# cristicbz/rust-doom

Measured on NVIDIA H100. Metric: frames/sec at 1920x1080 (palette-index bit-exact), higher is better.
Workload: dtype u8

## Files before the change

### rust-doom_b200/csrc/b2d_kernels.cu

```cuda
#include <type_traits>

#include "b2d_kernels.cuh"

namespace b2d {

namespace {

constexpr unsigned kFull = 0xFFFFFFFFu;

constexpr int kMaskWords = 128;
constexpr int kStackDepth = 128;

constexpr uint32_t kVisBit = 1u << 25, kSolidBit = 1u << 24;
__device__ __forceinline__ uint32_t pack_range(int lo, int hi, uint32_t bits) {
    return (uint32_t)lo | ((uint32_t)hi << 12) | bits;
}
__device__ __forceinline__ int range_lo(uint32_t r) { return (int)(r & 0xFFFu); }
__device__ __forceinline__ int range_hi(uint32_t r) { return (int)((r >> 12) & 0xFFFu); }

__device__ __forceinline__ uint32_t word_bits(int w, int lo, int hi) {
    int a = max(lo, w * 32), b = min(hi, w * 32 + 31);
    if (a > b) return 0u;
    uint32_t m = 0xFFFFFFFFu >> (31 - (b - w * 32));
    return m & (0xFFFFFFFFu << (a - w * 32));
// ... 331 lines not shown
    const uint8_t *texels, *flats;
    int row;
};

struct RasterCtx {
    const DeviceScene *sc;
    FixedWarp fix;
    uint32_t pal_s;
    uint2 *rowz;
    PlaneDir dir;
    uint8_t *fb;
    uint32_t *rgba;
    int W, H, x, lane;
    uint32_t skycol;
};

template <bool kRgba>
__device__ __forceinline__ void put_px(const RasterCtx &c, uint8_t *p8, uint32_t *p32, bool on, uint32_t v) {
    if (on) {
        if (kRgba) {
            *p8 = (uint8_t)v;
            *p32 = lds_u32(c.pal_s + 4u * v);
        } else {
            __stcs(p8, (uint8_t)v);
        }
    }
}

__host__ __device__ __forceinline__ bool tex_interleaved(const TexRec &T) { return b2d::tex_interleaved(T.h, T.texel_off); }

constexpr int kBatch = 8;

template <bool kRgba, int kW>
__device__ __forceinline__ void store_batch(const RasterCtx &c, uint8_t *p8, uint32_t *p32, const uint32_t (&v)[kBatch],
                                            int y, int ya, int yb, bool full) {
    const int Wc = kW ? kW : c.W;
    if (full) {
#pragma unroll
        for (int k = 0; k < kBatch; k++) put_px<kRgba>(c, p8 + (size_t)k * Wc, kRgba ? p32 + (size_t)k * Wc : nullptr, true, v[k]);
    } else {
        const uint32_t m = row_mask(y, ya, yb, kBatch);
#pragma unroll
        for (int k = 0; k < kBatch; k++)
            put_px<kRgba>(c, p8 + (size_t)k * Wc, kRgba ? p32 + (size_t)k * Wc : nullptr, (m >> k) & 1u, v[k]);
    }
}

template <bool kRgba, int kW>
__device__ __forceinline__ void fill_void_warp(const RasterCtx &c, int ya, int yb) {
    bool act = ya < yb;
    int y0 = __reduce_min_sync(kFull, act ? ya : 0x7FFFFFFF);
    int y1 = __reduce_max_sync(kFull, act ? yb : 0);
    if (y0 >= y1) return;
    const int Wc = kW ? kW : c.W;
    uint8_t *p8 = c.fb + (size_t)y0 * Wc;
    uint32_t *p32 = kRgba ? c.rgba + (size_t)y0 * Wc : nullptr;
#pragma unroll 1
    for (int y = y0; y < y1; y++, p8 += Wc, p32 += Wc) put_px<kRgba>(c, p8, p32, y >= ya && y < yb, 0u);
}

template <bool kRgba, int kW>
__device__ __forceinline__ void draw_sky_warp(const RasterCtx &c, int ya, int yb) {
    const DeviceScene &sc = *c.sc;
    if (sc.sky_tex < 0) { fill_void_warp<kRgba, kW>(c, ya, yb); return; }
    const TexRec T = sc.tex[sc.sky_tex];
    const bool inter = tex_interleaved(T);
    const uint8_t *px = sc.lit_texels + T.texel_off + (inter ? 4u * c.skycol : c.skycol);
    const uint32_t w4 = 4u * T.w;
    bool act = ya < yb;
    int y0 = __reduce_min_sync(kFull, act ? ya : 0x7FFFFFFF);
    int y1 = __reduce_max_sync(kFull, act ? yb : 0);
    if (y0 >= y1) return;
    const int Wc = kW ? kW : c.W;
    uint8_t *p8 = c.fb + (size_t)y0 * Wc;
    uint32_t *p32 = kRgba ? c.rgba + (size_t)y0 * Wc : nullptr;
#pragma unroll 2
    for (int y = y0; y < y1; y++, p8 += Wc, p32 += Wc) {
        const uint32_t r = sc.skyrow[y];
        put_px<kRgba>(c, p8, p32, y >= ya && y < yb, __ldg(px + (inter ? (r >> 2) * w4 + (r & 3u) : r * T.w)));
    }
}

template <bool kRgba, int kW, bool kFixed = false>
__device__ __forceinline__ void draw_plane_warp(const RasterCtx &c, const FrameConst &fc, const View &vw,
                                                int ya, int yb, int32_t h, int32_t flat, int lightb,
                                                bool visible) {
    const DeviceScene &sc = *c.sc;
    if (!__any_sync(kFull, ya < yb)) return;
    if (!visible) { fill_void_warp<kRgba, kW>(c, ya, yb); return; }
    if (flat == kFlatSky) { draw_sky_warp<kRgba, kW>(c, ya, yb); return; }
    if (flat < 0 || flat >= sc.nflats) { fill_void_warp<kRgba, kW>(c, ya, yb); return; }
    const uint8_t *lit_flats = sc.lit_flats;
    int fixed_row = -1;
    if constexpr (kFixed) {
        lit_flats = c.fix.row == 32 ? c.fix.flats : lit_flats;
        fixed_row = c.fix.row == 32 ? 0 : c.fix.row;
    }
    const uint64_t px_hi = reinterpret_cast<uint64_t>(lit_flats) & 0xFFFFFFFF00000000ull;
    const uint32_t habs = plane_habs(h, fc.pose.z);
    bool act = ya < yb;
    int y0 = __reduce_min_sync(kFull, act ? ya : 0x7FFFFFFF);
    int y1 = __reduce_max_sync(kFull, act ? yb : 0);
    const int full_lo = __reduce_max_sync(kFull, act ? ya : 0x7FFFFFFF);
    const int full_hi = __reduce_min_sync(kFull, act ? yb : 0);
    const int Wc = kW ? kW : c.W;
    uint8_t *p8 = c.fb + (size_t)y0 * Wc;
    uint32_t *p32 = kRgba ? c.rgba + (size_t)y0 * Wc : nullptr;
    const uint32_t bu = (uint32_t)fc.pose.x << 10, bv = (uint32_t)fc.pose.y << 10;
    const uint32_t ax = (uint32_t)c.dir.ax, ay = (uint32_t)c.dir.ay;
    for (int yc = y0; yc < y1; yc += 32) {
        int yy = yc + c.lane;
        if (yy < y1) {
            const PlaneRow pr = plane_row(habs, sc.yslope[yy]);
            c.rowz[c.lane] = make_uint2(pr.z8q, (sc.lit_flat_stride >> 6) * (uint32_t)(kFixed && fixed_row >= 0 ? fixed_row : light_row(lightb, pr.z8)) + 64u * (uint32_t)flat);
        }
        __syncwarp();
        const int rows = min(32, y1 - yc);
        int j = 0;
        for (; j + kBatch <= rows; j += kBatch, p8 += (size_t)kBatch * Wc, p32 += (size_t)kBatch * Wc) {
            uint32_t v[kBatch];
#pragma unroll
            for (int k = 0; k < kBatch; k++) {
                const uint2 rz = c.rowz[j + k];
                v[k] = __ldg(reinterpret_cast<const uint8_t *>(px_hi | flat_offset(rz.y, bu + rz.x * ax, bv + rz.x * ay)));
            }
            const int y = yc + j;
            store_batch<kRgba, kW>(c, p8, p32, v, y, ya, yb, y >= full_lo && y + kBatch <= full_hi);
        }
        for (; j < rows; j++, p8 += Wc, p32 += Wc) {
            const uint2 rz = c.rowz[j];
            const int y = yc + j;
            put_px<kRgba>(c, p8, p32, y >= ya && y < yb,
                          __ldg(reinterpret_cast<const uint8_t *>(px_hi | flat_offset(rz.y, bu + rz.x * ax, bv + rz.x * ay))));
        }
        __syncwarp();
    }
}

template <bool kRgba, int kW, int R>
__device__ __forceinline__ void wall_fast_loop(const RasterCtx &c, const uint8_t *plq, uint32_t w4, uint32_t nq, uint32_t q,
                                               uint32_t acc, uint32_t ts29, int y0, int y1, int ya, int yb,
                                               int full_lo, int full_hi) {
    const int Wc = kW ? kW : c.W;
    uint8_t *p8 = c.fb + (size_t)y0 * Wc;
    uint32_t *p32 = kRgba ? c.rgba + (size_t)y0 * Wc : nullptr;
    asm("" : "+l"(plq));
#pragma unroll 1
    for (int y = y0; y < y1; y += R, p8 += (size_t)R * Wc, p32 += (size_t)R * Wc) {
        const uint32_t q1 = q + 1u == nq ? 0u : q + 1u;
        const uint32_t w0 = __ldg(reinterpret_cast<const uint32_t *>(plq + (size_t)q * w4));
        const uint32_t w1 = __ldg(reinterpret_cast<const uint32_t *>(plq + (size_t)q1 * w4));
        if (y >= full_lo && y + R <= full_hi) {
#pragma unroll
            for (int k = 0; k < R; k++) {
                uint32_t v = pick_byte(w0, w1, wall_sel(acc, ts29, (uint32_t)k));
                if (kRgba) v &= 0xFFu;
                put_px<kRgba>(c, p8 + (size_t)k * Wc, kRgba ? p32 + (size_t)k * Wc : nullptr, true, v);
            }
        } else {
            const uint32_t m = row_mask(y, ya, yb, R);
#pragma unroll
            for (int k = 0; k < R; k++) {
                uint32_t v = pick_byte(w0, w1, wall_sel(acc, ts29, (uint32_t)k));
                if (kRgba) v &= 0xFFu;
                put_px<kRgba>(c, p8 + (size_t)k * Wc, kRgba ? p32 + (size_t)k * Wc : nullptr, (m >> k) & 1u, v);
            }
        }
        wall_advance(acc, q, ts29, (uint32_t)R, nq);
    }
}

template <bool kRgba, int kW, bool kFixed = false>
__device__ __forceinline__ void draw_wall_warp(const RasterCtx &c, const FrameConst &fc, int ya, int yb,
                                               int32_t tex, int32_t tA, int32_t hA, int32_t ucol,
                                               int32_t iscale, int row) {
    const DeviceScene &sc = *c.sc;
    if (!__any_sync(kFull, ya < yb)) return;
    if (tex < 0 || tex >= sc.ntex) { fill_void_warp<kRgba, kW>(c, ya, yb); return; }
    const TexRec T = sc.tex[tex];
    bool act = ya < yb;
    const uint32_t col = (uint32_t)floormod32(ucol, (int32_t)T.w);
    const uint8_t *pl = sc.lit_texels + (size_t)row * sc.lit_texel_stride + T.texel_off;
    if constexpr (kFixed) {
        if (row == 32) pl = c.fix.texels + T.texel_off;
    }
    const uint32_t tstep = (uint32_t)(iscale >> 4);
    int y0 = __reduce_min_sync(kFull, act ? ya : 0x7FFFFFFF);
    int y1 = __reduce_max_sync(kFull, act ? yb : 0);
    const int full_lo = __reduce_max_sync(kFull, act ? ya : 0x7FFFFFFF);
    const int full_hi = __reduce_min_sync(kFull, act ? yb : 0);
    uint32_t t = (uint32_t)wall_tbase(tA, hA, fc.pose.z, c.H, iscale) + (uint32_t)y0 * tstep;
    const int Wc = kW ? kW : c.W;
    uint8_t *p8 = c.fb + (size_t)y0 * Wc;
    uint32_t *p32 = kRgba ? c.rgba + (size_t)y0 * Wc : nullptr;
    if (tex_interleaved(T) && T.h >= 8u) {
        const uint32_t ts = act ? tstep : 0u;
        const bool f16 = __all_sync(kFull, ts <= kWallFast16);
        if (f16 || __all_sync(kFull, ts <= kWallFast8)) {
            const uint32_t tt = act ? t : 0u;
            const uint32_t r0 = wall_row((int32_t)tt, T.h, T.hmagic, T.hbias);
            const uint8_t *plq = pl + 4u * col;
            if (f16) wall_fast_loop<kRgba, kW, 16>(c, plq, 4u * T.w, T.h >> 2, r0 >> 2, wall_acc29(tt, r0), ts << 13, y0, y1, ya, yb, full_lo, full_hi);
            else wall_fast_loop<kRgba, kW, 8>(c, plq, 4u * T.w, T.h >> 2, r0 >> 2, wall_acc29(tt, r0), ts << 13, y0, y1, ya, yb, full_lo, full_hi);
            return;
        }
    }
    if (tex_interleaved(T)) {
        const uint32_t colb = 4u * col, w4 = 4u * T.w;
        for (int y = y0; y < y1; y += kBatch, p8 += (size_t)kBatch * Wc, p32 += (size_t)kBatch * Wc, t += (uint32_t)kBatch * tstep) {
            const uint32_t r0 = wall_row((int32_t)t, T.h, T.hmagic, T.hbias);
            const uint32_t acc = wall_acc(t, r0);
            const uint32_t b7 = (acc + 7u * tstep) >> 16;
            uint32_t v[kBatch];
            if (__all_sync(kFull, b7 < 8u)) {
                const uint32_t q0 = r0 >> 2, q1 = next_quad(q0, T.h);
                const uint32_t w0 = __ldg(reinterpret_cast<const uint32_t *>(pl + (q0 * w4 + colb)));
                const uint32_t w1 = __ldg(reinterpret_cast<const uint32_t *>(pl + (q1 * w4 + colb)));
#pragma unroll
                for (int k = 0; k < kBatch; k++) {
                    v[k] = pick_byte(w0, w1, (acc + (uint32_t)k * tstep) >> 16);
                    if (kRgba) v[k] &= 0xFFu;
                }
            } else {
                const uint32_t t4 = t + 4u * tstep;
                const uint32_t r4 = wall_row((int32_t)t4, T.h, T.hmagic, T.hbias);
                const uint32_t acc4 = wall_acc(t4, r4);
                if (__all_sync(kFull, ((acc + 3u * tstep) >> 16) < 8u && ((acc4 + 3u * tstep) >> 16) < 8u)) {
                    const uint32_t q0 = r0 >> 2, q4 = r4 >> 2;
                    const uint32_t a0 = __ldg(reinterpret_cast<const uint32_t *>(pl + (q0 * w4 + colb)));
                    const uint32_t a1 = __ldg(reinterpret_cast<const uint32_t *>(pl + (next_quad(q0, T.h) * w4 + colb)));
                    const uint32_t b0 = __ldg(reinterpret_cast<const uint32_t *>(pl + (q4 * w4 + colb)));
                    const uint32_t b1 = __ldg(reinterpret_cast<const uint32_t *>(pl + (next_quad(q4, T.h) * w4 + colb)));
#pragma unroll
                    for (int k = 0; k < 4; k++) {
                        v[k] = pick_byte(a0, a1, (acc + (uint32_t)k * tstep) >> 16);
                        v[k + 4] = pick_byte(b0, b1, (acc4 + (uint32_t)k * tstep) >> 16);
                        if (kRgba) { v[k] &= 0xFFu; v[k + 4] &= 0xFFu; }
                    }
                } else {
#pragma unroll
                    for (int k = 0; k < kBatch; k++) {
                        const uint32_t rk = wall_row((int32_t)(t + (uint32_t)k * tstep), T.h, T.hmagic, T.hbias);
                        v[k] = __ldg(pl + ((rk >> 2) * w4 + colb + (rk & 3u)));
                    }
                }
            }
            store_batch<kRgba, kW>(c, p8, p32, v, y, ya, yb, y >= full_lo && y + kBatch <= full_hi);
        }
    } else {
        const uint8_t *px = pl + col;
#pragma unroll 1
        for (int y = y0; y < y1; y++, p8 += Wc, p32 += Wc, t += tstep)
            put_px<kRgba>(c, p8, p32, y >= ya && y < yb, __ldg(px + wall_row((int32_t)t, T.h, T.hmagic, T.hbias) * T.w));
    }
}

__device__ __forceinline__ uint32_t *masked_entry(const DeviceScene &sc, const uint32_t *chunks, int e) {
    return sc.masked_list + ((size_t)chunks[e / kMaskedChunk] * kMaskedChunk + (size_t)(e % kMaskedChunk)) * 33u;
}
__device__ __forceinline__ uint32_t *masked_push(const DeviceScene &sc, uint32_t *chunks, int &mcount, int lane) {
    bool ok = mcount < sc.masked_cap;
    if (ok && mcount % kMaskedChunk == 0) {
        uint32_t id = 0;
        if (lane == 0) id = atomicAdd(sc.masked_counter, 1u);
        id = __shfl_sync(kFull, id, 0);
        ok = id < sc.masked_chunks;
        if (ok && lane == 0) chunks[mcount / kMaskedChunk] = id;
        __syncwarp();
    }
    if (!ok) {
        if (lane == 0) atomicOr(sc.status_flag, kStatusMaskedFull);
        return nullptr;
    }
    return masked_entry(sc, chunks, mcount++);
}

template <bool kRgba, int kW, bool kStates, bool kLevels, typename... Fix>
__device__ __noinline__ void masked_pass(const DeviceScene &sc, const View &vw, int32_t pose_z, uint8_t *fb,
                                         uint32_t *rgba, uint32_t pal_s, int x, int lane,
                                         const SegFrame *wl, const uint32_t *chunks, int count, Fix... fix) {
    constexpr bool kFixed = sizeof...(Fix) != 0;
    static_assert(sizeof...(Fix) == 0 || sizeof...(Fix) == 2, "the fixed colormap: the row-32 texel plane and the row");
    struct { const uint8_t *texels; int row; } const fw{fix...};
    RasterCtx c;
    c.sc = &sc; c.pal_s = pal_s; c.fb = fb; c.rgba = rgba;
    c.W = vw.W; c.H = vw.H; c.x = x; c.lane = lane;
    const int Wc = kW ? kW : c.W;
    for (int e = count - 1; e >= 0; e--) {
        const uint32_t *ml = masked_entry(sc, chunks, e);
        const uint32_t k = ml[0];
        const uint32_t packed = ml[1 + c.lane];
        int ya = (int)(packed & 0xFFFFu), yb = (int)(packed >> 16);
        const SegFrame sf = wl[k];
        int32_t tex, tA, hA, ucol = 0, iscale = 1, row = 0;
        if (is_sprite_entry(sf)) {
            SpriteFrame sp;
            const SpriteRec P = sc.sprites[entry_sprite(sf, sp)];
            if (P.tex < 0 || P.tex >= sc.ntex) continue;
            const int32_t sw = (int32_t)sc.tex[P.tex].w, sh = (int32_t)sc.tex[P.tex].h;
            const int64_t scale = sprite_scale(vw, sp.cz);
            int32_t z8;
            scale_depth(vw, scale, iscale, z8);
            row = kFixed && fw.row >= 0 ? fw.row : light_row_sprite(P.light, z8);
            tex = P.tex; tA = 0; hA = P.low + sh;
            if (ya < yb) {
                clip_rows(P.low + sh, P.low, row_scale(scale), pose_z, c.H, ya, yb);
                ucol = sprite_column(sp, vw, c.x, sw);
            }
        } else {
            const SegRec S = sc.segs[sf.seg];
            if (S.mid < 0 || S.mid >= sc.nmids) continue;
            const MidRec M = sc.mids[S.mid];
            tex = M.tex; tA = M.t_high; hA = M.high;
            ColumnEval ce = {0u, 1, 1, 0};
            if (ya < yb && column_eval(sf, vw, c.x, ce)) {
                clip_rows(M.high, M.low, ce.scale, pose_z, c.H, ya, yb);
                ucol = wall_column(S.uoff, S.len_q12, ce.s24);
                iscale = ce.iscale;
                row = kFixed && fw.row >= 0 ? fw.row : light_row(S.light, ce.z8);
            } else {
                ya = yb = 0;
            }
        }
        if (tex < 0 || tex >= sc.ntex) continue;
        const TexRec T = sc.tex[tex];
        const bool act = ya < yb;
        int y0 = __reduce_min_sync(kFull, act ? ya : 0x7FFFFFFF);
        int y1 = __reduce_max_sync(kFull, act ? yb : 0);
        if (y0 >= y1) continue;
        const uint32_t col = (uint32_t)floormod32(ucol, (int32_t)T.w);
        const bool inter = tex_interleaved(T);
        const bool has_mask = T.mask_off != 0xFFFFFFFFu;
        const uint8_t *pl = sc.lit_texels + (size_t)row * sc.lit_texel_stride + T.texel_off;
        if constexpr (kFixed) {
            if (row == 32) pl = fw.texels + T.texel_off;
        }
        const uint8_t *pm = sc.lit_texels + (size_t)32 * sc.lit_texel_stride + T.texel_off;
        const uint32_t tstep = (uint32_t)(iscale >> 4);
        uint32_t t = (uint32_t)wall_tbase(tA, hA, pose_z, c.H, iscale) + (uint32_t)y0 * tstep;
        uint8_t *p8 = c.fb + (size_t)y0 * Wc;
        uint32_t *p32 = kRgba ? c.rgba + (size_t)y0 * Wc : nullptr;
        const uint32_t len = act ? (uint32_t)(yb - ya) : 0u;
        if (inter) {
            const uint32_t colb = 4u * col, w4 = 4u * T.w;
#pragma unroll 1
            for (int y = y0; y < y1; y += kBatch, p8 += (size_t)kBatch * Wc, p32 += (size_t)kBatch * Wc, t += (uint32_t)kBatch * tstep) {
                const uint32_t r0 = wall_row((int32_t)t, T.h, T.hmagic, T.hbias);
                const uint32_t acc = wall_acc(t, r0);
                const uint32_t d = (uint32_t)(y - ya);
                uint32_t v[kBatch], o[kBatch];
                if (__all_sync(kFull, ((acc + 7u * tstep) >> 16) < 8u)) {
                    const uint32_t o0 = (r0 >> 2) * w4 + colb, o1 = next_quad(r0 >> 2, T.h) * w4 + colb;
                    const uint32_t w0 = __ldg(reinterpret_cast<const uint32_t *>(pl + o0));
                    const uint32_t w1 = __ldg(reinterpret_cast<const uint32_t *>(pl + o1));
                    uint32_t m0 = 0x01010101u, m1 = 0x01010101u;
                    if (has_mask) {
                        m0 = __ldg(reinterpret_cast<const uint32_t *>(pm + o0));
                        m1 = __ldg(reinterpret_cast<const uint32_t *>(pm + o1));
                    }
#pragma unroll
                    for (int k = 0; k < kBatch; k++) {
                        const uint32_t bk = (acc + (uint32_t)k * tstep) >> 16;
                        v[k] = pick_byte(w0, w1, bk) & 0xFFu;
                        o[k] = pick_byte(m0, m1, bk) & 0xFFu;
                    }
                } else {
#pragma unroll
                    for (int k = 0; k < kBatch; k++) {
                        const uint32_t rk = wall_row((int32_t)(t + (uint32_t)k * tstep), T.h, T.hmagic, T.hbias);
                        const uint32_t off = (rk >> 2) * w4 + colb + (rk & 3u);
                        v[k] = __ldg(pl + off);
                        o[k] = has_mask ? (uint32_t)__ldg(pm + off) : 1u;
                    }
                }
#pragma unroll
                for (int k = 0; k < kBatch; k++)
                    put_px<kRgba>(c, p8 + (size_t)k * Wc, kRgba ? p32 + (size_t)k * Wc : nullptr, d + (uint32_t)k < len && o[k] != 0u, v[k]);
            }
        } else {
#pragma unroll 1
            for (int y = y0; y < y1; y++, p8 += Wc, p32 += Wc, t += tstep) {
                const uint32_t off = wall_row((int32_t)t, T.h, T.hmagic, T.hbias) * T.w + col;
                const bool on = (uint32_t)(y - ya) < len && (!has_mask || __ldg(pm + off) != 0);
                put_px<kRgba>(c, p8, p32, on, __ldg(pl + off));
            }
        }
    }
}

constexpr int kRasterWarps = 8;

constexpr uint32_t kQueueWords = 6144;
constexpr uint32_t kQueueRecs = kQueueWords / 32;
constexpr uint32_t kRecWall = 1u << 16, kRecVisible = 1u << 17;

constexpr int kBandRows = 256;
constexpr int kMaxBands = (2160 + kBandRows - 1) / kBandRows;
constexpr uint32_t kItemCap = 1024;
static_assert(kBandRows % 32 == 0 && kMaxBands <= 256 && kQueueRecs <= 256, "an item is record | band << 8 in 16 bits");

struct DrawQueue {
    uint4 *head;
    uint32_t *ext;
    uint32_t *pool;
    uint32_t *nrec, *nwords;
};

__device__ __forceinline__ bool queue_push(const DrawQueue &q, int lane, uint32_t meta, int32_t a, int32_t b, int32_t c,
                                           int ya, int yb, int32_t ucol, uint32_t iscale_row) {
    const bool act = ya < yb;
    if (!__any_sync(kFull, act)) return true;
    const uint32_t y0 = __reduce_min_sync(kFull, act ? (uint32_t)ya : 0xFFFFu);
    const uint32_t y1 = __reduce_max_sync(kFull, act ? (uint32_t)yb : 0u);
    const bool wall = meta & kRecWall;
    const uint32_t words = wall ? 96u : 32u;
    uint32_t off = 0, i = kQueueRecs;
    if (lane == 0) {
        off = atomicAdd(q.nwords, words);
        if (off + words <= kQueueWords) i = atomicAdd(q.nrec, 1u);
    }
    i = __shfl_sync(kFull, i, 0);
    if (i >= kQueueRecs) return false;
    off = __shfl_sync(kFull, off, 0);
    q.pool[off + lane] = act ? (uint32_t)ya | ((uint32_t)yb << 16) : 0u;
    if (wall) {
        q.pool[off + 32 + lane] = (uint32_t)ucol;
        q.pool[off + 64 + lane] = iscale_row;
    }
    if (lane == 0) {
        q.head[i] = make_uint4(meta | off, (uint32_t)a, (uint32_t)b, (uint32_t)c);
        q.ext[i] = y0 | y1 << 16;
    }
    return true;
}

template <typename T, typename A, typename... P>
__device__ __forceinline__ const T &extra_tables(const A &a, const P &...p) {
    if constexpr (std::is_same_v<T, A>) return a;
    else return extra_tables<T>(p...);
}

template <bool kRgba, int kW, bool kMasked, bool kStates, bool kLevels, typename... Extra>
__global__ void __launch_bounds__(32 * kRasterWarps, 16 / kRasterWarps)
b2d_raster_kernel(const __grid_constant__ DeviceScene sc, const __grid_constant__ View vw, const FrameConst *__restrict__ frames,
                  const SegFrame *__restrict__ work, int stride, int n, int strips,
                  uint8_t *__restrict__ index_fb, uint32_t *__restrict__ rgba_fb, const __grid_constant__ LevelTables lt,
                  const Extra... fx) {
    constexpr bool kFixed = (std::is_same_v<Extra, FixedTables> || ...);
    constexpr bool kSeen = (std::is_same_v<Extra, SeenTables> || ...);
    static_assert(sizeof...(Extra) == (int)kFixed + (int)kSeen, "appended tables: FixedTables, SeenTables, each at most once");
    static_assert(!kFixed || (kStates && kLevels), "fixed colormaps come with per-frame levels and states");
    static_assert(!kSeen || !kRgba, "the seen variant draws index frames only");
    __shared__ uint32_t s_pal[kRgba ? (kLevels ? 256 * kRasterWarps : 256) : 1];
    __shared__ uint2 s_rowz[kRasterWarps][32];
    __shared__ uint32_t s_chunks[kRasterWarps][kMasked ? kMaskedCapMax / kMaskedChunk : 1];
    __shared__ int4 s_lanes[kRasterWarps][32];
    __shared__ int s_frame[kRasterWarps];
    __shared__ uint4 s_qhead[kQueueRecs];
    __shared__ uint32_t s_qext[kQueueRecs];
    __shared__ uint32_t s_qpool[kQueueWords];
    __shared__ uint16_t s_items[kItemCap];
    __shared__ uint32_t s_band[kMaxBands];
    __shared__ uint32_t s_qn[5];
    __shared__ DeviceScene s_scn[kStates || kLevels ? kRasterWarps : 1];
    __shared__ FixedWarp s_fix[kFixed ? kRasterWarps : 1];
    if (threadIdx.x < 5) s_qn[threadIdx.x] = 0;
    for (int b = threadIdx.x; b < kMaxBands; b += blockDim.x) s_band[b] = 0;
    if (kRgba && !kLevels) {
        for (int i = threadIdx.x; i < 256; i += blockDim.x) s_pal[i] = sc.palette[i];
    }
    __syncthreads();

    const int lane = threadIdx.x & 31, warp = threadIdx.x >> 5;
    const long long gw = (long long)blockIdx.x * (blockDim.x >> 5) + warp;
    const bool has_strip = gw < (long long)n * strips;
    const int frame = has_strip ? (int)(gw / strips) : 0, strip = has_strip ? (int)(gw % strips) : 0;
    const int W = kW ? kW : vw.W, H = vw.H;
    const int x0 = strip * 32, x = x0 + lane;
    const bool inside = has_strip && x < W;
    const DrawQueue q{s_qhead, s_qext, s_qpool, &s_qn[0], &s_qn[1]};

    FrameConst fc{};
    if (has_strip) fc = frames[frame];
    const DeviceScene *scp = &sc;
    if constexpr (kStates || kLevels) {
        DeviceScene *d = &s_scn[warp];
        if (has_strip) {
            const DeviceScene *lsrc = kLevels ? lt.scenes + (uint32_t)fc.level : &sc;
            const uint32_t *src = reinterpret_cast<const uint32_t *>(lsrc);
            uint32_t *dst = reinterpret_cast<uint32_t *>(d);
            for (int i = lane; i < (int)(sizeof(DeviceScene) / 4); i += 32) dst[i] = src[i];
            if (kLevels && kRgba) {
                const uint32_t *pal = lsrc->palette;
                for (int i = lane; i < 256; i += 32) s_pal[256 * warp + i] = pal[i];
            }
            __syncwarp();
            if constexpr (kStates) {
                if (lane == 0) {
                    const TableSet t = lt.sets[(uint32_t)fc.set];
                    d->tex = t.tex; d->sectors = t.sectors; d->segs = t.segs; d->sprites = t.sprites; d->mids = t.mids;
                }
                __syncwarp();
            }
        }
        scp = d;
    }
    if constexpr (kFixed) {
        if (has_strip && lane == 0) {
            const FixedTables &t = extra_tables<FixedTables>(fx...);
            const FixedPlanes p = t.planes[(uint32_t)fc.level];
            s_fix[warp] = FixedWarp{p.texels, p.flats, t.frame_fixed[frame]};
        }
        __syncwarp();
    }
    const DeviceScene &ts = *scp;
    const DeviceScene &ls = kLevels ? ts : sc;
    RasterCtx c;
    c.sc = &ts;
    if constexpr (kFixed) c.fix = s_fix[warp];
    c.pal_s = (uint32_t)__cvta_generic_to_shared(kLevels ? s_pal + 256 * warp : s_pal);
    c.rowz = s_rowz[warp];
    c.W = W; c.H = H; c.x = x; c.lane = lane;
    int mcount = 0;
    uint32_t *chunks = s_chunks[warp];
    asm("" : "+l"(chunks));
    const SegFrame *wl = work + (size_t)frame * stride;

    if (has_strip) {
    c.dir = plane_dir(fc, vw, inside ? x : 0, ls.invF);
    c.fb = index_fb + (size_t)frame * W * H + (inside ? x : 0);
    c.rgba = kRgba ? rgba_fb + (size_t)frame * W * H + (inside ? x : 0) : nullptr;
    c.skycol = 0;
    if (ls.sky_tex >= 0 && inside) c.skycol = umulhi32(sky_u32(x, vw, fc.pose.angle), ts.tex[ls.sky_tex].w);
    s_lanes[warp][lane] = make_int4(c.dir.ax, c.dir.ay, (int)c.skycol, inside ? x : 0);
    if (lane == 0) s_frame[warp] = frame;

    int ct = 0, cb = inside ? H : 0;
    const bool defer = kMasked && ls.masked_list != nullptr;
    const int count = fc.count;
    const uint32_t owner = (uint32_t)warp << 18;
    bool done = false;
    uint32_t *seen_row = nullptr;
    const int32_t *seen_line = nullptr;
    int32_t seen_last = -1;
    if constexpr (kSeen) {
        const SeenTables &st = extra_tables<SeenTables>(fx...);
        seen_row = st.rows + (size_t)frame * st.words;
        seen_line = st.seg_line + st.level_off[kLevels ? (uint32_t)fc.level : 0u];
    }

    for (int k0 = 0; k0 < count && !done; k0 += 32) {
        int k = k0 + lane;
        bool overlap = false;
        if (k < count) {
            int xlo = wl[k].xlo, xhi = wl[k].xhi;
            overlap = xhi >= x0 && xlo <= x0 + 31;
        }
        unsigned m = __ballot_sync(kFull, overlap);
        while (m) {
            int j = __ffs(m) - 1;
            m &= m - 1;
            if (!__any_sync(kFull, ct < cb)) { done = true; break; }
            const SegFrame sf = wl[k0 + j];
            bool in = inside && ct < cb && x >= sf.xlo && x <= sf.xhi;
            if (!__any_sync(kFull, in)) continue;
            if (is_sprite_entry(sf)) {
                if (defer) {
                    uint32_t *ml = masked_push(ls, chunks, mcount, lane);
                    if (ml) {
                        if (lane == 0) ml[0] = (uint32_t)(k0 + j);
                        ml[1 + lane] = in ? ((uint32_t)ct | ((uint32_t)cb << 16)) : 0u;
                    }
                }
                continue;
            }
            ColumnEval ce = {0u, 1, 1, 0};
            bool ok = in && column_eval(sf, vw, x, ce);
            if (!__any_sync(kFull, ok)) continue;
            if constexpr (kSeen) {
                if (lane == 0) {
                    const int32_t l = __ldg(seen_line + sf.seg);
                    if (l >= 0 && l != seen_last) {
                        atomicOr(seen_row + (l >> 5), 1u << (l & 31));
                        seen_last = l;
                    }
                }
            }

            const SegRec S = ts.segs[sf.seg];
            const SectorRec SF = ts.sectors[S.front];
            const int32_t fcl = SF.ceil, ffl = SF.floor;
            const bool two = S.flags & kSegTwoSided;
            const bool ceil_vis = plane_visible(true, fcl, SF.ceil_flat == kFlatSky, fc.pose.z);
            const bool floor_vis = plane_visible(false, ffl, SF.floor_flat == kFlatSky, fc.pose.z);

            WallRows wr = {ct, ct, ct, ct};
            int yend = ct, row = 0;
            int32_t ucol = 0;
            if (ok) {
                row = kFixed && c.fix.row >= 0 ? c.fix.row : light_row(S.light, ce.z8);
                ucol = wall_column(S.uoff, S.len_q12, ce.s24);
                wr = wall_rows(fcl, ffl, two, S.otop, S.obot, ce.scale, fc.pose.z, H, ct, cb);
                yend = cb;
            }
#pragma unroll 1
            for (int pz = 0; pz < 2; pz++) {
                const bool top = pz == 0;
                const int ya = ok ? (top ? ct : wr.y4) : 0, yb = ok ? (top ? wr.y1 : yend) : 0;
                const int32_t h = top ? fcl : ffl, flat = top ? SF.ceil_flat : SF.floor_flat;
                const bool vis = top ? ceil_vis : floor_vis;
                if (!queue_push(q, lane, owner | (vis ? kRecVisible : 0u), h, flat, SF.light, ya, yb, 0, 0u))
                    draw_plane_warp<kRgba, kW, kFixed>(c, fc, vw, ya, yb, h, flat, SF.light, vis);
            }
#pragma unroll 1
            for (int pw = 0; pw < 2; pw++) {
                const bool upper = pw == 0;
                if (!wall_piece(upper, two, fcl, ffl, S.otop, S.obot)) continue;
                const int ya = ok ? (upper ? wr.y1 : wr.y3) : 0, yb = ok ? (upper ? wr.y2 : wr.y4) : 0;
                const int32_t tex = upper ? S.texA : S.texB, tA = upper ? S.tA : S.tB, hA = upper ? S.hA : S.hB;
                if (!queue_push(q, lane, owner | kRecWall, tex, tA, hA, ya, yb, ucol, (uint32_t)ce.iscale | ((uint32_t)row << 24)))
                    draw_wall_warp<kRgba, kW, kFixed>(c, fc, ya, yb, tex, tA, hA, ucol, ce.iscale, row);
            }
            if (ok) wall_window(two, wr, H, ct, cb);
            if (defer && two && S.mid >= 0) {
                const bool keep = ok && wr.y2 < wr.y3;
                if (__any_sync(kFull, keep)) {
                    uint32_t *ml = masked_push(ls, chunks, mcount, lane);
                    if (ml) {
                        if (lane == 0) ml[0] = (uint32_t)(k0 + j);
                        ml[1 + lane] = keep ? ((uint32_t)wr.y2 | ((uint32_t)wr.y3 << 16)) : 0u;
                    }
                }
            }
        }
    }
    if (!queue_push(q, lane, owner, 0, 0, 0, inside ? ct : 0, inside ? cb : 0, 0, 0u))
        fill_void_warp<kRgba, kW>(c, inside ? ct : 0, inside ? cb : 0);
    }

    if (kMasked && mcount > 0 && lane == 0) s_qn[4] = 1;
    __syncthreads();
    const uint32_t nrec = min(s_qn[0], kQueueRecs);
    for (uint32_t r = threadIdx.x; r < nrec; r += blockDim.x) {
        const uint32_t e = s_qext[r];
        for (uint32_t b = (e & 0xFFFFu) / kBandRows; b <= ((e >> 16) - 1u) / kBandRows; b++) atomicAdd(&s_band[b], 1u);
    }
    __syncthreads();
    if (warp == 0) {
        constexpr int kPer = (kMaxBands + 31) / 32;
        uint32_t v[kPer], sum = 0;
#pragma unroll
        for (int k = 0; k < kPer; k++) {
            const int b = lane * kPer + k;
            v[k] = b < kMaxBands ? s_band[b] : 0u;
            sum += v[k];
        }
        uint32_t incl = sum;
#pragma unroll
        for (int d = 1; d < 32; d <<= 1) {
            const uint32_t u = __shfl_up_sync(kFull, incl, d);
            if (lane >= d) incl += u;
        }
        uint32_t at = incl - sum;
#pragma unroll
        for (int k = 0; k < kPer; k++) {
            const int b = lane * kPer + k;
            if (b < kMaxBands) s_band[b] = at;
            at += v[k];
        }
        if (lane == 31) s_qn[3] = incl;
    }
    __syncthreads();
    const bool banded = s_qn[3] <= kItemCap && !(kMasked && s_qn[4]);
    if (banded) {
        for (uint32_t r = threadIdx.x; r < nrec; r += blockDim.x) {
            const uint32_t e = s_qext[r];
            for (uint32_t b = (e & 0xFFFFu) / kBandRows; b <= ((e >> 16) - 1u) / kBandRows; b++)
                s_items[atomicAdd(&s_band[b], 1u)] = (uint16_t)(r | b << 8);
        }
        __syncthreads();
    }
    const uint32_t nitems = banded ? s_qn[3] : nrec;
    for (;;) {
        uint32_t i = 0;
        if (lane == 0) i = atomicAdd(&s_qn[2], 1u);
        i = __shfl_sync(kFull, i, 0);
        if (i >= nitems) break;
        int lo = 0, hi = H;
        if (banded) {
            const uint32_t it = s_items[i];
            i = it & 0xFFu;
            lo = (int)(it >> 8) * kBandRows;
            hi = lo + kBandRows;
        }
        const uint4 hd = s_qhead[i];
        const uint32_t off = hd.x & 0xFFFFu, o = hd.x >> 18;
        const int4 ln = s_lanes[o][lane];
        const int f = s_frame[o];
        const FrameConst fo = frames[f];
        RasterCtx d;
        d.sc = kStates || kLevels ? &s_scn[o] : &sc;
        if constexpr (kFixed) d.fix = s_fix[o];
        d.pal_s = (uint32_t)__cvta_generic_to_shared(kLevels ? s_pal + 256 * o : s_pal);
        d.rowz = s_rowz[warp];
        d.dir = PlaneDir{ln.x, ln.y};
        d.fb = index_fb + (size_t)f * W * H + ln.w;
        d.rgba = kRgba ? rgba_fb + (size_t)f * W * H + ln.w : nullptr;
        d.W = W; d.H = H; d.x = ln.w; d.lane = lane;
        d.skycol = (uint32_t)ln.z;
        const uint32_t win = s_qpool[off + lane];
        const int ya = max((int)(win & 0xFFFFu), lo), yb = min((int)(win >> 16), hi);
        if (hd.x & kRecWall) {
            const uint32_t isr = s_qpool[off + 64 + lane];
            draw_wall_warp<kRgba, kW, kFixed>(d, fo, ya, yb, (int32_t)hd.y, (int32_t)hd.z, (int32_t)hd.w, (int32_t)s_qpool[off + 32 + lane],
                                      (int32_t)(isr & 0xFFFFFFu), (int)(isr >> 24));
        } else {
            draw_plane_warp<kRgba, kW, kFixed>(d, fo, vw, ya, yb, (int32_t)hd.y, (int32_t)hd.z, (int)hd.w, hd.x & kRecVisible);
        }
    }
    if constexpr (kMasked) {
        __syncthreads();
        if constexpr (kFixed) {
            if (mcount > 0) masked_pass<kRgba, kW, kStates, kLevels>(ts, vw, fc.pose.z, c.fb, c.rgba, c.pal_s, x, lane, wl, chunks, mcount, c.fix.texels, c.fix.row);
        } else {
            if (mcount > 0) masked_pass<kRgba, kW, kStates, kLevels>(ts, vw, fc.pose.z, c.fb, c.rgba, c.pal_s, x, lane, wl, chunks, mcount);
        }
    }
}

__global__ void __launch_bounds__(256)
b2d_palette_kernel(const uint32_t *__restrict__ palette, const uint8_t *__restrict__ index,
                   uint32_t *__restrict__ rgba, size_t n_pixels) {
    __shared__ uint32_t s_pal[256];
    s_pal[threadIdx.x] = palette[threadIdx.x];
    __syncthreads();
    const bool aligned = ((reinterpret_cast<uintptr_t>(index) | reinterpret_cast<uintptr_t>(rgba)) & 15) == 0;
    const size_t nvec = aligned ? n_pixels / 16 : 0;
    const size_t stride = (size_t)gridDim.x * blockDim.x;
    for (size_t i = (size_t)blockIdx.x * blockDim.x + threadIdx.x; i < nvec; i += stride) {
        uint4 in = __ldcs(reinterpret_cast<const uint4 *>(index) + i);
        uint32_t wds[4] = {in.x, in.y, in.z, in.w};
        uint4 *out = reinterpret_cast<uint4 *>(rgba) + 4 * i;
#pragma unroll
        for (int q = 0; q < 4; q++) {
            uint4 o;
            o.x = s_pal[wds[q] & 0xFF];
            o.y = s_pal[(wds[q] >> 8) & 0xFF];
            o.z = s_pal[(wds[q] >> 16) & 0xFF];
            o.w = s_pal[wds[q] >> 24];
            __stcs(out + q, o);
        }
    }
    for (size_t p = nvec * 16 + (size_t)blockIdx.x * blockDim.x + threadIdx.x; p < n_pixels; p += stride)
        rgba[p] = s_pal[index[p]];
}

__global__ void __launch_bounds__(256)
b2d_palette_levels_kernel(const uint32_t *__restrict__ palettes, const uint32_t *__restrict__ tables,
                          const uint8_t *__restrict__ index, uint32_t *__restrict__ rgba, size_t npix, int parts) {
    __shared__ uint32_t s_pal[256];
    const size_t frame = blockIdx.x / parts;
    const int part = blockIdx.x % parts;
    s_pal[threadIdx.x] = palettes[(size_t)tables[frame] * 256 + threadIdx.x];
    __syncthreads();
    const uint8_t *in = index + frame * npix;
    uint32_t *out = rgba + frame * npix;
    const bool aligned = npix % 16 == 0 && ((reinterpret_cast<uintptr_t>(index) | reinterpret_cast<uintptr_t>(rgba)) & 15) == 0;
    const size_t n = aligned ? npix / 16 : npix;
    const size_t per = (n + parts - 1) / parts, lo = (size_t)part * per, hi = lo + per < n ? lo + per : n;
    if (aligned) {
        for (size_t i = lo + threadIdx.x; i < hi; i += blockDim.x) {
            const uint4 q = __ldcs(reinterpret_cast<const uint4 *>(in) + i);
            const uint32_t wds[4] = {q.x, q.y, q.z, q.w};
            uint4 *o4 = reinterpret_cast<uint4 *>(out) + 4 * i;
#pragma unroll
            for (int k = 0; k < 4; k++) {
                uint4 o;
                o.x = s_pal[wds[k] & 0xFF];
                o.y = s_pal[(wds[k] >> 8) & 0xFF];
                o.z = s_pal[(wds[k] >> 16) & 0xFF];
                o.w = s_pal[wds[k] >> 24];
                __stcs(o4 + k, o);
            }
        }
    } else {
        for (size_t p = lo + threadIdx.x; p < hi; p += blockDim.x) out[p] = s_pal[in[p]];
    }
}

constexpr int kResolveRgba = 0, kResolveRgb = 1, kResolvePlanar = 2, kResolveGray = 3;

template <int N>
__device__ __forceinline__ void store_run(uint8_t *dst, const uint32_t (&w)[(N + 3) / 4]) {
    const uintptr_t a = reinterpret_cast<uintptr_t>(dst);
    if constexpr (N % 16 == 0) {
        if ((a & 15) == 0) {
#pragma unroll
            for (int q = 0; q < N / 16; q++) __stcs(reinterpret_cast<uint4 *>(dst) + q, make_uint4(w[4 * q], w[4 * q + 1], w[4 * q + 2], w[4 * q + 3]));
            return;
        }
// ... 536 lines not shown
```

### rust-doom_b200/csrc/b2d_math.cuh

```cuda
#pragma once
#include <stdint.h>

#if defined(__CUDACC__)
#define B2D_HD __host__ __device__ __forceinline__
#else
#define B2D_HD inline
#endif

namespace b2d {

struct Pose { int32_t x, y, z; uint32_t angle; };
struct View { int32_t W, H, F, FY2; };

struct FrameConst {
    Pose pose;
    int32_t cosq, sinq;
    int32_t px8, py8;
    int32_t count;
    int32_t status;
    int32_t set;
    int32_t level;
    int32_t pad[4];
};
static_assert(sizeof(FrameConst) == 64, "FrameConst");
// ... 213 lines not shown
    r.y1 = clampv(yfc, ct, cb);
    if (!two) {
        r.y2 = clampv(yff, r.y1, cb);
        r.y3 = r.y2; r.y4 = r.y2;
    } else {
        r.y2 = clampv(yrow(otop, scale, pose_z, H), r.y1, cb);
        r.y3 = clampv(yrow(obot, scale, pose_z, H), r.y2, cb);
        r.y4 = clampv(yff, r.y3, cb);
    }
    return r;
}
B2D_HD bool wall_piece(bool upper, bool two, int32_t ceil, int32_t floor, int32_t otop, int32_t obot) {
    return upper ? (!two || otop < ceil) : (two && obot > floor);
}
B2D_HD void wall_window(bool two, const WallRows &r, int32_t H, int &ct, int &cb) {
    if (!two || r.y2 >= r.y3) { ct = H; cb = 0; }
    else { ct = r.y2; cb = r.y3; }
}
B2D_HD int32_t wall_column(int32_t uoff, int32_t len_q12, uint32_t s24) {
    return uoff + (int32_t)(((uint64_t)s24 * (uint32_t)len_q12) >> 36);
}
B2D_HD void clip_rows(int32_t high, int32_t low, int32_t scale, int32_t pose_z, int32_t H, int &ya, int &yb) {
    const int a = yrow(high, scale, pose_z, H), b = yrow(low, scale, pose_z, H);
    if (a > ya) ya = a;
    if (b < yb) yb = b;
}

B2D_HD uint32_t yslope_entry(int y, const View &vw) {
    int32_t r2 = 2 * y + 1 - vw.H;
    if (r2 < 0) r2 = -r2;
    if (r2 == 0) r2 = 1;
    const uint64_t s = ((uint64_t)vw.FY2 << 16) / (uint32_t)r2;
    return s > 0xFFFFFFFFull ? 0xFFFFFFFFu : (uint32_t)s;
}

B2D_HD uint32_t plane_habs(int32_t h, int32_t pose_z) {
    int64_t hrel = clampv<int64_t>(((int64_t)h << 16) - pose_z, -((int64_t)1 << 27), (int64_t)1 << 27);
    return (uint32_t)(hrel < 0 ? -hrel : hrel);
}
B2D_HD int32_t wall_hrel(int32_t h, int32_t pose_z) {
    return (int32_t)clampv<int64_t>(((int64_t)h << 16) - pose_z, -((int64_t)1 << 27), (int64_t)1 << 27);
}

struct PlaneDir { int32_t ax, ay; };
B2D_HD PlaneDir plane_dir(const FrameConst &f, const View &vw, int x, uint32_t invF) {
    const int64_t c2 = 2 * (int64_t)x + 1 - vw.W;
    const int64_t nx = ((int64_t)f.cosq * vw.F + (int64_t)f.sinq * c2) >> 4;
    const int64_t ny = ((int64_t)f.sinq * vw.F - (int64_t)f.cosq * c2) >> 4;
    const int64_t m = (int64_t)invF << 24;
    PlaneDir d;
#if defined(__CUDA_ARCH__)
    d.ax = (int32_t)__mul64hi(nx, m);
    d.ay = (int32_t)__mul64hi(ny, m);
#else
    d.ax = (int32_t)(int64_t)(((__int128)nx * m) >> 64);
    d.ay = (int32_t)(int64_t)(((__int128)ny * m) >> 64);
#endif
    return d;
}
struct PlaneRow { uint32_t z8q; int32_t z8; };
B2D_HD PlaneRow plane_row(uint32_t habs, uint32_t yslope) {
    PlaneRow pr;
    uint64_t zz = ((uint64_t)habs * yslope) >> 16;
    int32_t z16 = zz > 0x7FFFFFFFull ? 0x7FFFFFFF : (int32_t)zz;
    pr.z8q = (uint32_t)(z16 >> 8);
    int32_t z8 = z16 >> 13;
    pr.z8 = z8 > 65535 ? 65535 : z8;
    return pr;
}
B2D_HD uint32_t plane_u(int32_t pose_xy, uint32_t z8q, int32_t a) { return ((uint32_t)pose_xy << 10) + z8q * (uint32_t)a; }
B2D_HD uint32_t flat_index(uint32_t U, uint32_t V) { return ((U >> 26) << 6) | (V >> 26); }
B2D_HD uint32_t flat_offset(uint32_t cm6, uint32_t U, uint32_t V) {
#if defined(__CUDA_ARCH__)
    return __funnelshift_l(V, cm6 + (U >> 26), 6);
#else
    return ((cm6 + (U >> 26)) << 6) | (V >> 26);
#endif
}

B2D_HD int32_t wall_tbase(int32_t tA, int32_t hA, int32_t pose_z, int32_t H, int32_t iscale) {
    int64_t t = ((int64_t)tA << 16) + wall_hrel(hA, pose_z) + (((int64_t)(1 - H) * iscale) >> 5);
    return (int32_t)t;
}
B2D_HD uint32_t wall_row(int32_t t, uint32_t h, uint32_t hmagic, uint32_t hbias) {
    uint32_t n = ((uint32_t)t + (hbias << 16)) >> 16;
    uint32_t q = umulhi32(n, hmagic);
    const uint32_t r = n - q * h;
    return r < h ? r : 0u;
}

B2D_HD bool tex_interleaved(uint32_t h, uint32_t texel_off) { return (h & 3u) == 0u && (texel_off & 3u) == 0u && h <= 4096u; }
B2D_HD uint32_t lit_index(bool inter, uint32_t w, uint32_t row, uint32_t col) {
    return inter ? ((row >> 2) * w + col) * 4u + (row & 3u) : row * w + col;
}
B2D_HD uint32_t wall_acc(uint32_t t, uint32_t r0) { return (t & 0xFFFFu) | ((r0 & 3u) << 16); }
B2D_HD uint32_t next_quad(uint32_t q0, uint32_t h) { return q0 + 1u == (h >> 2) ? 0u : q0 + 1u; }
B2D_HD uint32_t pick_byte(uint32_t lo, uint32_t hi, uint32_t sel) {
#if defined(__CUDA_ARCH__)
    uint32_t d;
    asm("prmt.b32 %0, %1, %2, %3;" : "=r"(d) : "r"(lo), "r"(hi), "r"(sel));
    return d;
#else
    return ((sel & 4u) ? hi : lo) >> (8u * (sel & 3u)) & 0xFFu;
#endif
}

constexpr uint32_t kWallFast8 = 32768u;
constexpr uint32_t kWallFast16 = 16384u;
B2D_HD uint32_t wall_acc29(uint32_t t, uint32_t r0) { return ((r0 & 3u) << 29) | ((t & 0xFFFFu) << 13); }
B2D_HD uint32_t wall_sel(uint32_t acc, uint32_t ts29, uint32_t k) { return (acc + k * ts29) >> 29; }
B2D_HD void wall_advance(uint32_t &acc, uint32_t &q, uint32_t ts29, uint32_t R, uint32_t nq) {
    acc += R * ts29;
    q += acc >> 31;
    if (q >= nq) q -= nq;
    acc &= 0x7FFFFFFFu;
}
B2D_HD uint32_t row_mask(int y, int ya, int yb, int R) {
    int lo = ya - y, hi = yb - y;
    if (lo < 0) lo = 0;
    if (hi > R) hi = R;
    if (hi <= lo) return 0u;
    return ((1u << hi) - 1u) & ~((1u << lo) - 1u);
}

B2D_HD uint32_t sky_u32(int x, const View &vw, uint32_t angle) {
    uint64_t num = ((uint64_t)(2 * x + 1)) << 32;
    return (uint32_t)(num / (uint32_t)vw.W) - (angle << 3);
}
B2D_HD int32_t sky_row(int y, int32_t H, int32_t skyh) {
    int32_t r = 2 * y + 1;
    if (r < H) return (r * skyh) / H;
    return floormod32(((2 * H - r) * skyh) / H, skyh);
}

constexpr int32_t kBoxNearQ8 = 32 * 256;
B2D_HD bool box_range(const FrameConst &f, const View &vw, const int32_t box[4], int &lo, int &hi) {
    bool all_behind = true, any_near = false;
    int64_t mn = 0x7FFFFFFFFFFFFFFFLL, mx = -0x7FFFFFFFFFFFFFFFLL;
    for (int i = 0; i < 4; i++) {
        int32_t tx, tz;
        to_view(f, box[2 + (i & 1)], box[i >> 1], tx, tz);
        if (tz >= -256) all_behind = false;
        if (tz < kBoxNearQ8) { any_near = true; continue; }
        int64_t c = floordiv64((int64_t)tx * vw.F, tz);
        int64_t xc = floordiv64(c - 1 + vw.W, 2);
        if (xc < mn) mn = xc;
        if (xc > mx) mx = xc;
    }
    if (all_behind) return false;
    if (any_near) { lo = 0; hi = vw.W - 1; return true; }
    mn -= 2; mx += 2;
    if (mx < 0 || mn > vw.W - 1) return false;
    lo = (int)(mn < 0 ? 0 : mn);
    hi = (int)(mx > vw.W - 1 ? vw.W - 1 : mx);
    return true;
}

B2D_HD int light_row_sprite(int b, int32_t z8) {
    int32_t r1 = (32 * (255 - b)) / 255;
    uint32_t Z = (uint32_t)z8 + 800u;
    int32_t num = (int32_t)(64u * (uint32_t)(255 - b) * Z) - 6528000;
    int32_t r2 = num <= 0 ? 0 : (int32_t)((uint32_t)num / (255u * Z));
    int32_t r = r1 > r2 ? r1 : r2;
    return r > 31 ? 31 : r;
}

// ... 271 lines not shown
```

Baseline: 619,000.

## Precompute wall texture setup per queued record and halve band rows

```diff
diff --git a/rust-doom_b200/csrc/b2d_kernels.cu b/rust-doom_b200/csrc/b2d_kernels.cu
--- a/rust-doom_b200/csrc/b2d_kernels.cu
+++ b/rust-doom_b200/csrc/b2d_kernels.cu
@@ -437,8 +437,8 @@
 }
 
 template <bool kRgba, int kW, bool kFixed = false>
-__device__ __forceinline__ void draw_plane_warp(const RasterCtx &c, const FrameConst &fc, const View &vw,
-                                                int ya, int yb, int32_t h, int32_t flat, int lightb,
+__device__ __forceinline__ void draw_plane_warp(const RasterCtx &c, int32_t pose_x, int32_t pose_y,
+                                                int ya, int yb, uint32_t habs, int32_t flat, int lightb,
                                                 bool visible) {
     const DeviceScene &sc = *c.sc;
     if (!__any_sync(kFull, ya < yb)) return;
@@ -452,7 +452,6 @@
         fixed_row = c.fix.row == 32 ? 0 : c.fix.row;
     }
     const uint64_t px_hi = reinterpret_cast<uint64_t>(lit_flats) & 0xFFFFFFFF00000000ull;
-    const uint32_t habs = plane_habs(h, fc.pose.z);
     bool act = ya < yb;
     int y0 = __reduce_min_sync(kFull, act ? ya : 0x7FFFFFFF);
     int y1 = __reduce_max_sync(kFull, act ? yb : 0);
@@ -461,7 +460,7 @@
     const int Wc = kW ? kW : c.W;
     uint8_t *p8 = c.fb + (size_t)y0 * Wc;
     uint32_t *p32 = kRgba ? c.rgba + (size_t)y0 * Wc : nullptr;
-    const uint32_t bu = (uint32_t)fc.pose.x << 10, bv = (uint32_t)fc.pose.y << 10;
+    const uint32_t bu = (uint32_t)pose_x << 10, bv = (uint32_t)pose_y << 10;
     const uint32_t ax = (uint32_t)c.dir.ax, ay = (uint32_t)c.dir.ay;
     for (int yc = y0; yc < y1; yc += 32) {
         int yy = yc + c.lane;
@@ -525,16 +524,33 @@
     }
 }
 
+struct WallSetup {
+    uint32_t texel_off, tpiece, hmagic, w, h, path;
+};
+constexpr uint32_t kWallPathR8 = 2u, kWallPathR16 = 3u;
+
+__device__ __forceinline__ WallSetup wall_setup(const DeviceScene &sc, int32_t tex, int32_t tA, int32_t hA, int32_t pose_z,
+                                                bool act, uint32_t tstep) {
+    const TexRec T = sc.tex[tex];
+    uint32_t path = tex_interleaved(T) ? 1u : 0u;
+    if (path && T.h >= 8u) {
+        const uint32_t ts = act ? tstep : 0u;
+        if (__all_sync(kFull, ts <= kWallFast16)) path = kWallPathR16;
+        else if (__all_sync(kFull, ts <= kWallFast8)) path = kWallPathR8;
+    }
+    return WallSetup{T.texel_off, wall_tpiece(tA, hA, pose_z) + (T.hbias << 16), T.hmagic, T.w, T.h, path};
+}
+__device__ __forceinline__ uint32_t wall_setup_word(const WallSetup &T) { return T.w | T.h << 13 | T.path << 26; }
+__device__ __forceinline__ WallSetup wall_setup_at(uint4 hd, uint32_t word) {
+    return WallSetup{hd.y, hd.z, hd.w, word & 0x1FFFu, (word >> 13) & 0x1FFFu, word >> 26};
+}
+
 template <bool kRgba, int kW, bool kFixed = false>
-__device__ __forceinline__ void draw_wall_warp(const RasterCtx &c, const FrameConst &fc, int ya, int yb,
-                                               int32_t tex, int32_t tA, int32_t hA, int32_t ucol,
-                                               int32_t iscale, int row) {
+__device__ __forceinline__ void draw_wall_warp(const RasterCtx &c, const WallSetup &T, int ya, int yb,
+                                               uint32_t col, int32_t iscale, int row) {
     const DeviceScene &sc = *c.sc;
     if (!__any_sync(kFull, ya < yb)) return;
-    if (tex < 0 || tex >= sc.ntex) { fill_void_warp<kRgba, kW>(c, ya, yb); return; }
-    const TexRec T = sc.tex[tex];
     bool act = ya < yb;
-    const uint32_t col = (uint32_t)floormod32(ucol, (int32_t)T.w);
     const uint8_t *pl = sc.lit_texels + (size_t)row * sc.lit_texel_stride + T.texel_off;
     if constexpr (kFixed) {
         if (row == 32) pl = c.fix.texels + T.texel_off;
@@ -544,26 +560,23 @@
     int y1 = __reduce_max_sync(kFull, act ? yb : 0);
     const int full_lo = __reduce_max_sync(kFull, act ? ya : 0x7FFFFFFF);
     const int full_hi = __reduce_min_sync(kFull, act ? yb : 0);
-    uint32_t t = (uint32_t)wall_tbase(tA, hA, fc.pose.z, c.H, iscale) + (uint32_t)y0 * tstep;
+    uint32_t t = T.tpiece + wall_tcol(c.H, iscale) + (uint32_t)y0 * tstep;
     const int Wc = kW ? kW : c.W;
     uint8_t *p8 = c.fb + (size_t)y0 * Wc;
     uint32_t *p32 = kRgba ? c.rgba + (size_t)y0 * Wc : nullptr;
-    if (tex_interleaved(T) && T.h >= 8u) {
+    if (T.path >= kWallPathR8) {
         const uint32_t ts = act ? tstep : 0u;
-        const bool f16 = __all_sync(kFull, ts <= kWallFast16);
-        if (f16 || __all_sync(kFull, ts <= kWallFast8)) {
-            const uint32_t tt = act ? t : 0u;
-            const uint32_t r0 = wall_row((int32_t)tt, T.h, T.hmagic, T.hbias);
-            const uint8_t *plq = pl + 4u * col;
-            if (f16) wall_fast_loop<kRgba, kW, 16>(c, plq, 4u * T.w, T.h >> 2, r0 >> 2, wall_acc29(tt, r0), ts << 13, y0, y1, ya, yb, full_lo, full_hi);
-            else wall_fast_loop<kRgba, kW, 8>(c, plq, 4u * T.w, T.h >> 2, r0 >> 2, wall_acc29(tt, r0), ts << 13, y0, y1, ya, yb, full_lo, full_hi);
-            return;
-        }
-    }
-    if (tex_interleaved(T)) {
+        const uint32_t tt = act ? t : 0u;
+        const uint32_t r0 = wall_row((int32_t)tt, T.h, T.hmagic, 0u);
+        const uint8_t *plq = pl + 4u * col;
+        if (T.path == kWallPathR16) wall_fast_loop<kRgba, kW, 16>(c, plq, 4u * T.w, T.h >> 2, r0 >> 2, wall_acc29(tt, r0), ts << 13, y0, y1, ya, yb, full_lo, full_hi);
+        else wall_fast_loop<kRgba, kW, 8>(c, plq, 4u * T.w, T.h >> 2, r0 >> 2, wall_acc29(tt, r0), ts << 13, y0, y1, ya, yb, full_lo, full_hi);
+        return;
+    }
+    if (T.path) {
         const uint32_t colb = 4u * col, w4 = 4u * T.w;
         for (int y = y0; y < y1; y += kBatch, p8 += (size_t)kBatch * Wc, p32 += (size_t)kBatch * Wc, t += (uint32_t)kBatch * tstep) {
-            const uint32_t r0 = wall_row((int32_t)t, T.h, T.hmagic, T.hbias);
+            const uint32_t r0 = wall_row((int32_t)t, T.h, T.hmagic, 0u);
             const uint32_t acc = wall_acc(t, r0);
             const uint32_t b7 = (acc + 7u * tstep) >> 16;
             uint32_t v[kBatch];
@@ -578,7 +591,7 @@
                 }
             } else {
                 const uint32_t t4 = t + 4u * tstep;
-                const uint32_t r4 = wall_row((int32_t)t4, T.h, T.hmagic, T.hbias);
+                const uint32_t r4 = wall_row((int32_t)t4, T.h, T.hmagic, 0u);
                 const uint32_t acc4 = wall_acc(t4, r4);
                 if (__all_sync(kFull, ((acc + 3u * tstep) >> 16) < 8u && ((acc4 + 3u * tstep) >> 16) < 8u)) {
                     const uint32_t q0 = r0 >> 2, q4 = r4 >> 2;
@@ -595,7 +608,7 @@
                 } else {
 #pragma unroll
                     for (int k = 0; k < kBatch; k++) {
-                        const uint32_t rk = wall_row((int32_t)(t + (uint32_t)k * tstep), T.h, T.hmagic, T.hbias);
+                        const uint32_t rk = wall_row((int32_t)(t + (uint32_t)k * tstep), T.h, T.hmagic, 0u);
                         v[k] = __ldg(pl + ((rk >> 2) * w4 + colb + (rk & 3u)));
                     }
                 }
@@ -606,7 +619,7 @@
         const uint8_t *px = pl + col;
 #pragma unroll 1
         for (int y = y0; y < y1; y++, p8 += Wc, p32 += Wc, t += tstep)
-            put_px<kRgba>(c, p8, p32, y >= ya && y < yb, __ldg(px + wall_row((int32_t)t, T.h, T.hmagic, T.hbias) * T.w));
+            put_px<kRgba>(c, p8, p32, y >= ya && y < yb, __ldg(px + wall_row((int32_t)t, T.h, T.hmagic, 0u) * T.w));
     }
 }
 
@@ -749,7 +762,7 @@
 constexpr uint32_t kQueueRecs = kQueueWords / 32;
 constexpr uint32_t kRecWall = 1u << 16, kRecVisible = 1u << 17;
 
-constexpr int kBandRows = 256;
+constexpr int kBandRows = 128;
 constexpr int kMaxBands = (2160 + kBandRows - 1) / kBandRows;
 constexpr uint32_t kItemCap = 1024;
 static_assert(kBandRows % 32 == 0 && kMaxBands <= 256 && kQueueRecs <= 256, "an item is record | band << 8 in 16 bits");
@@ -810,8 +823,9 @@
     __shared__ uint2 s_rowz[kRasterWarps][32];
     __shared__ uint32_t s_chunks[kRasterWarps][kMasked ? kMaskedCapMax / kMaskedChunk : 1];
     __shared__ int4 s_lanes[kRasterWarps][32];
-    __shared__ int s_frame[kRasterWarps];
+    __shared__ int4 s_own[kRasterWarps];
     __shared__ uint4 s_qhead[kQueueRecs];
+    __shared__ uint32_t s_qtex[kQueueRecs];
     __shared__ uint32_t s_qext[kQueueRecs];
     __shared__ uint32_t s_qpool[kQueueWords];
     __shared__ uint16_t s_items[kItemCap];
@@ -888,7 +902,7 @@
     c.skycol = 0;
     if (ls.sky_tex >= 0 && inside) c.skycol = umulhi32(sky_u32(x, vw, fc.pose.angle), ts.tex[ls.sky_tex].w);
     s_lanes[warp][lane] = make_int4(c.dir.ax, c.dir.ay, (int)c.skycol, inside ? x : 0);
-    if (lane == 0) s_frame[warp] = frame;
+    if (lane == 0) s_own[warp] = make_int4(frame, fc.pose.x, fc.pose.y, fc.pose.z);
 
     int ct = 0, cb = inside ? H : 0;
     const bool defer = kMasked && ls.masked_list != nullptr;
@@ -965,7 +979,7 @@
                 const int32_t h = top ? fcl : ffl, flat = top ? SF.ceil_flat : SF.floor_flat;
                 const bool vis = top ? ceil_vis : floor_vis;
                 if (!queue_push(q, lane, owner | (vis ? kRecVisible : 0u), h, flat, SF.light, ya, yb, 0, 0u))
-                    draw_plane_warp<kRgba, kW, kFixed>(c, fc, vw, ya, yb, h, flat, SF.light, vis);
+                    draw_plane_warp<kRgba, kW, kFixed>(c, fc.pose.x, fc.pose.y, ya, yb, plane_habs(h, fc.pose.z), flat, SF.light, vis);
             }
 #pragma unroll 1
             for (int pw = 0; pw < 2; pw++) {
@@ -973,8 +987,14 @@
                 if (!wall_piece(upper, two, fcl, ffl, S.otop, S.obot)) continue;
                 const int ya = ok ? (upper ? wr.y1 : wr.y3) : 0, yb = ok ? (upper ? wr.y2 : wr.y4) : 0;
                 const int32_t tex = upper ? S.texA : S.texB, tA = upper ? S.tA : S.tB, hA = upper ? S.hA : S.hB;
-                if (!queue_push(q, lane, owner | kRecWall, tex, tA, hA, ya, yb, ucol, (uint32_t)ce.iscale | ((uint32_t)row << 24)))
-                    draw_wall_warp<kRgba, kW, kFixed>(c, fc, ya, yb, tex, tA, hA, ucol, ce.iscale, row);
+                if (!queue_push(q, lane, owner | kRecWall, tex, tA, hA, ya, yb, ucol, (uint32_t)ce.iscale | ((uint32_t)row << 24))) {
+                    if (tex < 0 || tex >= ts.ntex) {
+                        fill_void_warp<kRgba, kW>(c, ya, yb);
+                    } else {
+                        const WallSetup T = wall_setup(ts, tex, tA, hA, fc.pose.z, ya < yb, (uint32_t)(ce.iscale >> 4));
+                        draw_wall_warp<kRgba, kW, kFixed>(c, T, ya, yb, (uint32_t)floormod32(ucol, (int32_t)T.w), ce.iscale, row);
+                    }
+                }
             }
             if (ok) wall_window(two, wr, H, ct, cb);
             if (defer && two && S.mid >= 0) {
@@ -996,6 +1016,27 @@
     if (kMasked && mcount > 0 && lane == 0) s_qn[4] = 1;
     __syncthreads();
     const uint32_t nrec = min(s_qn[0], kQueueRecs);
+    for (uint32_t r = warp; r < nrec; r += kRasterWarps) {
+        uint4 hd = s_qhead[r];
+        const uint32_t off = hd.x & 0xFFFFu, o = hd.x >> 18;
+        const int32_t pose_z = s_own[o].w;
+        const DeviceScene &rs = kStates || kLevels ? s_scn[o] : sc;
+        if (!(hd.x & kRecWall)) {
+            hd.y = plane_habs((int32_t)hd.y, pose_z);
+        } else if ((int32_t)hd.y < 0 || (int32_t)hd.y >= rs.ntex) {
+            hd.x &= ~(kRecWall | kRecVisible);
+        } else {
+            const uint32_t win = s_qpool[off + lane];
+            const bool act = (win & 0xFFFFu) < (win >> 16);
+            const WallSetup T = wall_setup(rs, (int32_t)hd.y, (int32_t)hd.z, (int32_t)hd.w, pose_z, act,
+                                           (s_qpool[off + 64 + lane] & 0xFFFFFFu) >> 4);
+            s_qpool[off + 32 + lane] = (uint32_t)floormod32((int32_t)s_qpool[off + 32 + lane], (int32_t)T.w);
+            hd = make_uint4(hd.x, T.texel_off, T.tpiece, T.hmagic);
+            if (lane == 0) s_qtex[r] = wall_setup_word(T);
+        }
+        __syncwarp();
+        if (lane == 0) s_qhead[r] = hd;
+    }
     for (uint32_t r = threadIdx.x; r < nrec; r += blockDim.x) {
         const uint32_t e = s_qext[r];
         for (uint32_t b = (e & 0xFFFFu) / kBandRows; b <= ((e >> 16) - 1u) / kBandRows; b++) atomicAdd(&s_band[b], 1u);
@@ -1051,8 +1092,8 @@
         const uint4 hd = s_qhead[i];
         const uint32_t off = hd.x & 0xFFFFu, o = hd.x >> 18;
         const int4 ln = s_lanes[o][lane];
-        const int f = s_frame[o];
-        const FrameConst fo = frames[f];
+        const int4 ow = s_own[o];
+        const int f = ow.x;
         RasterCtx d;
         d.sc = kStates || kLevels ? &s_scn[o] : &sc;
         if constexpr (kFixed) d.fix = s_fix[o];
@@ -1067,10 +1108,10 @@
         const int ya = max((int)(win & 0xFFFFu), lo), yb = min((int)(win >> 16), hi);
         if (hd.x & kRecWall) {
             const uint32_t isr = s_qpool[off + 64 + lane];
-            draw_wall_warp<kRgba, kW, kFixed>(d, fo, ya, yb, (int32_t)hd.y, (int32_t)hd.z, (int32_t)hd.w, (int32_t)s_qpool[off + 32 + lane],
-                                      (int32_t)(isr & 0xFFFFFFu), (int)(isr >> 24));
+            draw_wall_warp<kRgba, kW, kFixed>(d, wall_setup_at(hd, s_qtex[i]), ya, yb, s_qpool[off + 32 + lane],
+                                              (int32_t)(isr & 0xFFFFFFu), (int)(isr >> 24));
         } else {
-            draw_plane_warp<kRgba, kW, kFixed>(d, fo, vw, ya, yb, (int32_t)hd.y, (int32_t)hd.z, (int)hd.w, hd.x & kRecVisible);
+            draw_plane_warp<kRgba, kW, kFixed>(d, ow.y, ow.z, ya, yb, hd.y, (int32_t)hd.z, (int)hd.w, hd.x & kRecVisible);
         }
     }
     if constexpr (kMasked) {
diff --git a/rust-doom_b200/csrc/b2d_math.cuh b/rust-doom_b200/csrc/b2d_math.cuh
--- a/rust-doom_b200/csrc/b2d_math.cuh
+++ b/rust-doom_b200/csrc/b2d_math.cuh
@@ -319,6 +319,8 @@
     int64_t t = ((int64_t)tA << 16) + wall_hrel(hA, pose_z) + (((int64_t)(1 - H) * iscale) >> 5);
     return (int32_t)t;
 }
+B2D_HD uint32_t wall_tpiece(int32_t tA, int32_t hA, int32_t pose_z) { return ((uint32_t)tA << 16) + (uint32_t)wall_hrel(hA, pose_z); }
+B2D_HD uint32_t wall_tcol(int32_t H, int32_t iscale) { return (uint32_t)(((int64_t)(1 - H) * iscale) >> 5); }
 B2D_HD uint32_t wall_row(int32_t t, uint32_t h, uint32_t hmagic, uint32_t hbias) {
     uint32_t n = ((uint32_t)t + (hbias << 16)) >> 16;
     uint32_t q = umulhi32(n, hmagic);
```

Result: no change. 618,100, median of 6 (-0.1%).
